# jonathan-innis/karpenter-provider-aws

Hardware: AMD Instinct MI355X
Metric: pods scheduled/sec (Solve, 50k pods × EC2 catalog) (higher is better)
Workload: dtype int64; 1 GPU; config2: 50000 heterogeneous pods (250 classes) x 918 types x 3 AZ x {spot,on-demand}, 2 NodePools; pods=50000, types=918, parallelism=single

## Files before the change

karpenter-provider-aws_amd/csrc/kp_bound.h:

```cpp
#pragma once
#include <stdint.h>

#if defined(__HIPCC__) || defined(__CUDACC__)
#define KP_BOUND_HD __host__ __device__ inline
#else
#define KP_BOUND_HD inline
#endif

#define KP_BOUND_STRIDE 8
#define KP_NO_BOUND INT64_MAX

KP_BOUND_HD int64_t kp_bound_entry(int64_t max_alloc, bool witness) { return witness ? max_alloc : KP_NO_BOUND; }

KP_BOUND_HD bool kp_bound_rejects(int64_t bound, int64_t total, int64_t pod) {
    return pod > 0 && bound != KP_NO_BOUND && total > bound - pod;
}
```

karpenter-provider-aws_amd/csrc/kp_ffd.h:

```cpp
#pragma once
#include <hip/hip_runtime.h>
#include <stdint.h>

#include <type_traits>

#include "kp_bound.h"
#include "kp_device.h"
#include "kp_eval.h"
#include "kp_gosort.h"
#include "kp_layout.h"

namespace KP_WNS {

#ifdef KP_NO_TOPO
#define KP_TOPO_ON 0
#else
#define KP_TOPO_ON 1
#endif

__device__ __forceinline__ bool ports_meet(const KpDev& d, const uint64_t* m, int c) {
    uint64_t x = 0;
    for (int w = 0; w < d.PW; w++)
        x |= __hip_atomic_load(const_cast<uint64_t*>(m) + w, __ATOMIC_RELAXED, __HIP_MEMORY_SCOPE_AGENT) &
             d.cls_ports[(size_t)c * d.PW + w];
// ... 294 lines not shown
}

__device__ inline void topo_record_quick(const KpDev& d, FfdShared& S, int c, int nc, int tmpl, uint64_t born, int lane) {
    const bool hit = S.tr_cls == c;
    const int r0 = hit ? 0 : d.cls_troff[c], nr = hit ? S.tr_n : d.cls_troff[c + 1] - r0;
    const bool keep = !hit && nr <= KP_SNAP_ROWS;
    for (int base = 0; base < nr; base += 64) {
        const int i = base + lane;
        KpTopoRec R{};
        uint32_t fl = 0;
        uint64_t w = 0;
        bool live = false;
        if (i < nr) {
            R = hit ? S.tr_R[i] : d.cls_tre[r0 + i];
            if (keep) S.tr_R[i] = R;
            live = !((R.skip >> tmpl) & 1ull) && (R.late < 0 || ((born >> R.late) & 1ull));
            if (live && !(R.flags & 8)) {
                fl = d.nc_hdr[(size_t)nc * d.K + R.key].flags;
                w = d.nc_words[(size_t)nc * d.DW + d.woff[R.key]];
                const int type = R.flags & TG_TYPE;
                const bool inv = (R.flags >> 2) & 1;
                live = (fl & RF_DEF) && !(!inv && type != 2 && ((fl & RF_CMP) || __popcll(w) != 1));
            }
        }
        for (uint64_t m = ballot(live); m; m &= m - 1) {
            const int j = __ffsll((unsigned long long)m) - 1;
            const int g = rl32(R.g, j), flags = rl32(R.flags, j), key = rl32(R.key, j);
            if (flags & 8) {
                if (lane == 0) {
                    const int old = atomicAdd(&d.tg_hcnt[(size_t)(-1 - key) * d.HN + d.E + nc], 1);
                    if (old == 0) atomicAdd(&d.tg_pos[g], 1);
                }
                continue;
            }
            const uint64_t wv = rl64(w, j);
            if ((wv >> lane) & 1ull) atomicAdd(&d.tg_cnt[(size_t)g * 64 + lane], 1);
            if (lane == 0 && wv) atomicOr((unsigned long long*)&d.tg_known[g], (unsigned long long)wv);
        }
    }
    if (keep && lane == 0) {
        S.tr_n = nr;
        S.tr_cls = c;
    }
    asm volatile("s_waitcnt vmcnt(0)" ::: "memory");
}

#define KP_CAND_VIRT 0x40000000
#ifndef KP_BOUND_SWEEP
#define KP_BOUND_SWEEP 0
#endif
#ifndef KP_BOUND_IDLE_WAVE
#define KP_BOUND_IDLE_WAVE 1
#endif
template <bool PROF>
static __device__ __attribute__((noinline)) int bound_round(const int64_t* __restrict__ nc_bound,
                                                            const int64_t* __restrict__ nc_req,
                                                            int R, int A,
                                                            FfdShared& S, uint32_t* key, const uint16_t* ord, int buf,
                                                            int cnt, int sdone, int r) {
    static_assert(KP_NWAVES <= 8 && KP_LDS_AXES <= KP_BOUND_STRIDE && KP_BOUND_STRIDE == 8, "lane = 8 candidate + axis");
    const int lane = (int)__lane_id(), ci = lane >> 3, ai = lane & 7;
    const bool v = ci < cnt && ai < A;
    const int nc = ord[S.cand_pos[buf][ci < cnt ? ci : 0]];
    const int64_t b = v ? __hip_atomic_load(const_cast<int64_t*>(&nc_bound[(size_t)nc * KP_BOUND_STRIDE + ai]), __ATOMIC_RELAXED,
                                            __HIP_MEMORY_SCOPE_AGENT) : KP_NO_BOUND;
    const int64_t tot = v ? ld_req(&nc_req[(size_t)nc * R + r]) : 0;
    const uint64_t m = ballot(v && kp_bound_rejects(b, tot, S.pod_req[r]));
    if (!m) return 0;
    uint64_t vm = 0;
    for (int i = 0; i < 8; i++)
        if ((m >> (8 * i)) & 0xFFull) vm |= 1ull << i;
    const int nv = __popcll(vm);
    const int p = lane < cnt ? S.cand_pos[buf][lane] : 0;
    const bool rej = (vm >> lane) & 1ull;
    if (nv == cnt && !sdone) {
        if (rej) key[p] |= 0x80000000u;
        if (lane == 0) {
            S.st[ST_NC_EVALS] += cnt;
            S.st[ST_BOUND_SKIPS] += cnt;
            if (PROF) S.st[ST_BOUND_ALLV]++;
            S.fwd = 1;
        }
        return 1;
    }
    if (rej) S.cand_pos[buf][lane] = p | KP_CAND_VIRT;
    if (PROF && lane == 0) S.st[nv == cnt ? ST_BOUND_ALLV : ST_BOUND_MIXED]++;
    return 0;
}
template <bool TOPO, bool PORTS = false, bool BOUND = false, bool PROF = false>
__device__ inline bool collect_candidates(const KpDev& d, FfdShared& S,
                                          std::conditional_t<PORTS || BOUND, uint32_t*, const uint32_t*> key,
                                          const uint16_t* ord, const uint8_t* stmpl, uint64_t tol, int N, int start, int buf,
                                          int lane, int pc = -1, bool bound = false) {
    int pos = start;
    bool marked = false;
    for (;;) {
        int cnt = 0, next = N;
        const int tp_n = TOPO ? S.tp_n : 0;
        const int L = tp_n ? d.topo_cands : KP_NWAVES;
        while (pos < N) {
            const int p = pos + lane;
            bool c = p < N && !(key[p] >> 31);
            if (c) c = (tol >> stmpl[ord[p]]) & 1ull;
            if (PORTS && pc >= 0) {
                const bool meet = c && ports_meet(d, d.nc_ports + (size_t)ord[p] * d.PW, pc);
                if constexpr (PORTS)
                    if (meet) key[p] |= 0x80000000u;
                marked |= ballot(meet) != 0;
                c = c && !meet;
            }
            if (tp_n && c) c = topo_prefilter_pass(d, S, ord[p]);
            const uint64_t m0 = __ballot(c);
            if (tp_n && m0 && cnt + __popcll(m0) < L) {
                const int rank = cnt + __popcll(m0 & ((1ull << lane) - 1ull));
                if (c) S.cand_pos[buf][rank] = p;
                cnt += __popcll(m0);
                pos += 64;
                if (lane == 0) {
                    S.n_cand[buf] = cnt;
                    S.scan_next[buf] = pos < N ? pos : N;
                    S.scan_done[buf] = pos >= N;
                }
                return marked;
            }
            const uint64_t m = __ballot(c);
            const int rank = cnt + __popcll(m & ((1ull << lane) - 1ull));
            if (c && rank < L) S.cand_pos[buf][rank] = p;
            const int tot = cnt + __popcll(m);
            if (tot >= L) {
                const uint64_t last = __ballot(c && rank == L - 1);
                next = pos + __ffsll((unsigned long long)last);
                cnt = L;
                break;
            }
            cnt = tot;
            pos += 64;
        }
        const bool sdone = (cnt < L) || next >= N;
        if constexpr (BOUND) {
            if (bound && cnt > 0 && d.lds_A > 0) {
                __builtin_amdgcn_fence(__ATOMIC_SEQ_CST, "wavefront");
                if (bound_round<PROF>(d.nc_bound, d.nc_req, d.R, d.lds_A, S, key, ord,
                                            buf, cnt, sdone, act_axis(d, lane & 7))) {
                    marked = true;
                    pos = next;
                    continue;
                }
            }
        }
        if (lane == 0) {
            S.n_cand[buf] = cnt;
            S.scan_next[buf] = cnt == L ? next : N;
            S.scan_done[buf] = sdone;
        }
        return marked;
    }
}

static __device__ __attribute__((noinline)) void bound_row_store(const KpDev* __restrict__ dp, const int64_t* alloc,
                                                                 const WaveScratch& ws, int nc, int fresh) {
    static_assert(KP_LDS_AXES < KP_BOUND_STRIDE, "the row's last entry holds the walk's first step");
    const KpDev& d = *dp;
    const int lane = (int)__lane_id();
    const int A = d.lds_A, TP = d.lds_tpad;
    const uint16_t* const rank = d.alloc_rank;
    int64_t* const row = d.nc_bound + (size_t)nc * KP_BOUND_STRIDE;
    int64_t mx[KP_LDS_AXES];
#if KP_BOUND_SWEEP
    const int start = 0, first = 0;
    for (int ai = 0; ai < KP_LDS_AXES; ai++) {
        mx[ai] = KP_NO_BOUND;
        if (ai >= A) continue;
        int64_t m = INT64_MIN;
        for (int w = 0; w < d.TW; w++)
            if ((ws.opts[w] >> lane) & 1ull) {
                const int64_t av = alloc[ai * TP + w * 64 + lane];
                m = av > m ? av : m;
            }
        mx[ai] = wave_max64(m);
    }
#else
    int t[KP_LDS_AXES];
#pragma unroll
    for (int ai = 0; ai < KP_LDS_AXES; ai++) {
        mx[ai] = KP_NO_BOUND;
        t[ai] = ai < A ? (int)rank[ai * TP + lane] : 0xFFFF;
    }
    const int start = fresh ? 0 : (int)__hip_atomic_load(&row[KP_BOUND_STRIDE - 1], __ATOMIC_RELAXED, __HIP_MEMORY_SCOPE_AGENT);
    int base = start * 64;
    if (start > 0) {
#pragma unroll
        for (int ai = 0; ai < KP_LDS_AXES; ai++) t[ai] = ai < A ? (int)rank[ai * TP + base + lane] : 0xFFFF;
    }
    uint32_t pending = (1u << A) - 1u;
    int first = -1;
    while (base < TP) {
#pragma unroll
        for (int ai = 0; ai < KP_LDS_AXES; ai++)
            if ((pending >> ai) & 1u) {
                const uint64_t m = ballot(t[ai] < TP && ((ws.opts[t[ai] < TP ? t[ai] >> 6 : 0] >> (t[ai] & 63)) & 1ull));
                if (m) {
                    mx[ai] = alloc[ai * TP + rl32(t[ai], __ffsll((unsigned long long)m) - 1)];
                    pending &= ~(1u << ai);
                    if (first < 0) first = base >> 6;
                }
            }
        base += 64;
        if (!pending || base >= TP) break;
#pragma unroll
        for (int ai = 0; ai < KP_LDS_AXES; ai++) t[ai] = ((pending >> ai) & 1u) ? (int)rank[ai * TP + base + lane] : 0xFFFF;
    }
#endif
    int64_t mine = KP_NO_BOUND;
#pragma unroll
    for (int ai = 0; ai < KP_LDS_AXES; ai++)
        if (lane == ai) mine = mx[ai];
    if (lane < A)
        __hip_atomic_store(&row[lane], kp_bound_entry(mine, ws.hr[lane] >= 0), __ATOMIC_RELAXED, __HIP_MEMORY_SCOPE_AGENT);
    if (lane == KP_BOUND_STRIDE - 1)
        __hip_atomic_store(&row[lane], (int64_t)(first < 0 ? start : first), __ATOMIC_RELAXED, __HIP_MEMORY_SCOPE_AGENT);
}

__device__ __forceinline__ uint64_t limit_filter(const KpDev& d, int j, uint64_t o, int lane) {
    return lane < d.TW ? o & d.tmpl_lmask[(size_t)j * d.TW + lane] : o;
}

__device__ inline void limit_mask_update(const KpDev& d, int j, int lane) {
    uint32_t lm = 0;
    for (int r = 0; r < d.R; r++)
        if (d.limit_set[(size_t)j * d.R + r]) lm |= 1u << r;
    uint64_t mine = ~0ull;
    for (int w = 0; w < d.TW && lm; w++) {
        const int t = w * 64 + lane;
        bool keep = t < d.T;
        for (uint32_t m = lm; m && keep; m &= m - 1) {
            const int r = __ffs(m) - 1;
            keep = d.cap[(size_t)r * d.T + t] <= ld_req(&d.remaining[(size_t)j * d.R + r]);
        }
        const uint64_t nb = ballot(keep);
        if (lane == w) mine = nb;
    }
    if (lane < d.TW) d.tmpl_lmask[(size_t)j * d.TW + lane] = mine;
}

__device__ __forceinline__ long long prof_clock(bool prof) { return prof ? __builtin_amdgcn_s_memtime() : 0; }


__device__ __forceinline__ void commit_reservations(const KpDev& d, int32_t* rcap, const WaveScratch& ws, int nc,
                                                    bool fresh, int* rel_flag, int lane) {
    const int RW = d.ro_ridw;
    if (lane < RW) {
        uint64_t* hp = d.nc_held + (size_t)nc * RW + lane;
        const uint64_t old = fresh ? 0ull : ld_u64(hp), nh = ws.minbits[lane];
        for (uint64_t x = nh & ~old; x; x &= x - 1) rcap[lane * 64 + __ffsll((unsigned long long)x) - 1]--;
        for (uint64_t x = old & ~nh; x; x &= x - 1)
            if (rcap[lane * 64 + __ffsll((unsigned long long)x) - 1]++ == 0) *rel_flag = 1;
        __hip_atomic_store(hp, nh, __ATOMIC_RELAXED, __HIP_MEMORY_SCOPE_AGENT);
    }
    if (lane == 0) __hip_atomic_store(&d.nc_rlive[nc], ws.rlive, __ATOMIC_RELAXED, __HIP_MEMORY_SCOPE_AGENT);
}
__device__ __forceinline__ uint64_t held_word(const KpDev& d, int nc, int lane) {
    return lane < d.ro_ridw ? ld_u64(&d.nc_held[(size_t)nc * d.ro_ridw + lane]) : 0ull;
}

template <bool VOL = false>
static __device__ __attribute__((noinline)) int existing_topo_scan(const KpDev* __restrict__ dp, FfdShared& S, int pod, int lane) {
    const KpDev& d = *dp;
    const int K = d.K;
    const int c = S.cur_cls;
    int vs = 0;
    if constexpr (VOL)
        if (d.VD > 0) vs = __builtin_amdgcn_readfirstlane(d.shape_vs[d.pod_shape[pod]]);
    const bool cons = (d.cls_flags[c] & CF_TOPO_CONS) != 0;
// ... 1259 lines not shown
                    const int i = atomicAdd(&trace[0], 1);
                    {
                        int* e = trace + 1 + 6 * (i % KP_TRACE_N);
                        e[0] = pod;
                        e[1] = nc;
                        e[2] = ok;
                        e[3] = S.ws[wave].memo_ok | (fast << 1) | ((RESV ? ld_i32(&d.nc_rlive[nc]) : 0) << 2);
                        e[4] = S.cand_pos[b][ci];
                        e[5] = (int)(rl64(a.held, 0) & 0xFFFFFFFFu);
                    }
                }
                if (lane == 0) {
                    S.fastp[b][ci] = fast;
                    S.acc[b][ci] = ok;
                    if (!ok && S.ws[wave].memo_ok) {
                        skey[S.cand_pos[b][ci]] |= 0x80000000u;
                        S.any_rej = 1;
                    }
                    if (!ok && !S.ws[wave].memo_ok) S.rej_volatile = 1;
                    if (fast) atomicAdd((unsigned long long*)&S.st[ST_WITNESS_MISS], 1ull);
                }
            }
            __syncthreads();
            const int nc_ = S.n_cand[b];
            for (int w = f0; w < nc_; w++)
                if (S.acc[b][w]) {
                    win = w;
                    break;
                }
            if (tid == 0) S.st[ST_NC_EVALS] += nc_ > f0 ? nc_ - f0 : 0;
            if (win >= 0 || S.scan_done[b]) break;
            if (wave == 0 &&
                collect_candidates<TOPO_ON, PORTS, BOUND, PROF>(d, S, skey, sord, stmpl, S.topo_pod ? d.tol[S.cur_cls] : ~0ull, S.N,
                                                                      S.scan_next[b], b ^ 1, lane,
                                                                      (PORTS && (S.CC.flags & CF_PORTS)) ? S.cur_cls : -1,
                                                                      BOUND && !(S.CC.flags & CF_TOPO)) && lane == 0)
                S.any_rej = 1;
            __syncthreads();
            round++;
        }
        long long c_ev = 0;
        if (tid == 0 && prof) {
            const long long t1 = __builtin_amdgcn_s_memtime();
            S.st[ST_CYC_SCAN] += t1 - c_slow;
            S.st[ST_SEG + 3] += t1 - c_ev0;
            c_ev = t1;
        }
        if (prof && tid == 0 && !S.topo_pod)
            S.st[ST_SLOW_WHY + (win < 0 ? 7 : (round == 0 && win == 0) ? 5 : 6)]++;
        if (win >= 0) {
            const int cw = (team || team_won) ? 0 : win - (round == 0 ? first : 0);
            if (BOUND && wave == (cw + KP_BOUND_IDLE_WAVE) % KP_NWAVES)
            {
                bound_row_store(d.self, E.alloc, S.ws[(team || team_won) ? wave : cw], sord[S.cand_pos[round & 1][win]], 0);
                asm volatile("s_waitcnt vmcnt(0)" ::: "memory");
            }
            if (wave == cw) {
                const int pos = S.cand_pos[round & 1][win];
                const int nc = sord[pos];
                if (!S.fastp[round & 1][win]) {
                    commit_reqs(d, S.CC, S.ws[cw], nc, lane);
                    if (RESV && d.resv_on) commit_reservations(d, sRcap, S.ws[cw], nc, false, &S.rel_flag, lane);
                }
                if (PREF && d.best_effort) {
                    asm volatile("s_waitcnt vmcnt(0)" ::: "memory");
                    commit_min_relax(d, S.ws[cw], nc, lane);
                }
                if (TOPO_ON && (S.CC.flags & CF_TOPO))
                    topo_record(d, S.CC, S.ws[cw], d.nc_hdr + (size_t)nc * K, d.nc_words + (size_t)nc * d.DW,
                                d.E + nc, d.nc_tmpl[nc], true, lane, -1, nullptr, S.born);
                if (lane < TW) d.nc_opts[(size_t)nc * TW + lane] = S.ws[cw].opts[lane];
                if (PORTS && (S.CC.flags & CF_PORTS)) nodeclaim_ports_commit(d, nc, S.cur_cls, false, 0, lane);
                if (lane < R && S.pod_req[lane])
                    atomicAdd((unsigned long long*)&d.nc_req[(size_t)nc * R + lane], (unsigned long long)S.pod_req[lane]);
                if (lane < A && nc < NQ) shr[lane * NQ + nc] = S.ws[cw].hr[lane];
                if (lane == 0) {
                    slast[nc] = (uint16_t)S.cur_cls;
                    skey[pos]++;
                    S.dirty_kind = 1;
                    S.dirty_pos = pos;
                    S.scan_start = ((S.CC.flags & CF_TOPO) || S.rej_volatile) ? 0 : pos;
                    if (trace && S.cur_cls == -2 - d.trace_pod && pod <= d.trace_max) {
                        const int i = atomicAdd(&trace[0], 1);
                        {
                            int* e = trace + 1 + 6 * (i % KP_TRACE_N);
                            e[0] = pod;
                            e[1] = -1000 - nc;
                            e[2] = S.scan_start;
                            e[3] = S.rej_volatile;
                            e[4] = pos;
                            e[5] = 0;
                        }
                    }
                    d.pod_result[pod] = nc;
                    d.pod_order[pod] = S.seq++;
                }
                asm volatile("s_waitcnt vmcnt(0)" ::: "memory");
            }
        } else {
            const long long c_t = prof_clock(prof);
            auto commit_tmpl = [&](int jj, int cw) {
                const int n = S.N;
                for (int k = lane; k < K; k += 64) d.nc_hdr[(size_t)n * K + k] = d.cls_hdr[(size_t)(d.C + jj) * K + k];
                for (int i = lane; i < d.DW; i += 64)
                    d.nc_words[(size_t)n * d.DW + i] = d.cls_words[(size_t)(d.C + jj) * d.DW + i];
                asm volatile("s_waitcnt vmcnt(0)" ::: "memory");
                commit_reqs(d, S.CC, S.ws[cw], n, lane);
                if (PREF && d.best_effort) {
                    asm volatile("s_waitcnt vmcnt(0)" ::: "memory");
                    commit_min_relax(d, S.ws[cw], n, lane);
                }
                if (RESV && d.resv_on) commit_reservations(d, sRcap, S.ws[cw], n, true, &S.rel_flag, lane);
                if (TOPO_ON && (S.CC.flags & CF_TOPO))
                    topo_record(d, S.CC, S.ws[cw], d.cls_hdr + (size_t)(d.C + jj) * K,
                                d.cls_words + (size_t)(d.C + jj) * d.DW, d.E + n, jj, true, lane, -1, nullptr,
                                S.born);
                if (lane < TW) d.nc_opts[(size_t)n * TW + lane] = S.ws[cw].opts[lane];
                if (PORTS) nodeclaim_ports_commit(d, n, S.cur_cls, true, jj, lane);
                for (int r = lane; r < R; r += 64)
                    __hip_atomic_store(&d.nc_req[(size_t)n * R + r], d.daemon[(size_t)jj * R + r] + S.pod_req[r],
                                       __ATOMIC_RELAXED, __HIP_MEMORY_SCOPE_AGENT);
                if (lane < A && n < NQ) shr[lane * NQ + n] = S.ws[cw].hr[lane];
                if (BOUND) bound_row_store(d.self, E.alloc, S.ws[cw], n, 1);
                for (int r = 0; r < R; r++) {
                    if (!d.limit_set[(size_t)jj * R + r]) continue;
                    int64_t mx = INT64_MIN;
                    for (int w2 = 0; w2 < TW; w2++) {
                        const uint64_t ow = S.ws[cw].opts[w2];
                        if ((ow >> lane) & 1ull) {
                            const int64_t cp = d.cap[(size_t)r * T + w2 * 64 + lane];
                            mx = cp > mx ? cp : mx;
                        }
                    }
                    mx = wave_max64(mx);
                    if (lane == 0) d.remaining[(size_t)jj * R + r] -= mx;
                }
                asm volatile("s_waitcnt vmcnt(0)" ::: "memory");
                limit_mask_update(d, jj, lane);
                if (lane == 0) {
                    slast[n] = (uint16_t)S.cur_cls;
                    stmpl[n] = (uint8_t)jj;
                    d.nc_tmpl[n] = jj;
                    sord[n] = (uint16_t)n;
                    skey[n] = 1;
                    S.N = n + 1;
                    S.dirty_kind = 2;
                    S.dirty_pos = n;
                    d.pod_result[pod] = n;
                    d.pod_order[pod] = S.seq++;
                }
                asm volatile("s_waitcnt vmcnt(0)" ::: "memory");
            };
            int twin = -1;
            if (KP_TEAM_TMPL && (!RESV || KP_TEAM_TMPL_RESV) && !TOPO && d.team_first) {
                for (int j = 0; j < d.NT; j++) {
                    uint64_t o = (lane < TW && d.tmpl_ok[j]) ? d.tmpl_opts[(size_t)j * TW + lane] : 0;
                    o = limit_filter(d, j, o, lane);
                    if (PORTS && (S.CC.flags & CF_PORTS) && ports_meet(d, d.tmpl_ports + (size_t)j * d.PW, S.cur_cls)) o = 0;
                    if (!ballot(o != 0)) continue;
                    EvalIn a;
                    a.Ahdr = d.cls_hdr + (size_t)(d.C + j) * K;
                    a.Aw = d.cls_words + (size_t)(d.C + j) * d.DW;
                    a.opts = o;
                    a.base_req = d.daemon + (size_t)j * R;
                    a.pod_req = S.pod_req;
                    a.tmpl = j;
                    a.compat = true;
                    a.force_off = false;
                    a.prof = nullptr;
                    a.host = d.E + S.N;
                    a.held = 0;
                    TeamBuf* const tbuf = &S.team[tjoins & 1];
                    const bool ok = (TOPO_ON && (S.CC.flags & CF_TOPO_CONS))
                                        ? eval_wave<true, RESV, true, PREF, false, true, PROF>(d, E, S.CC, a, S.ws[wave], lane, tbuf,
                                                                                         wave, KP_NWAVES, &tjoins)
                                        : eval_wave<false, RESV, true, PREF, false, true, PROF>(d, E, S.CC, a, S.ws[wave], lane,
                                                                                          tbuf, wave, KP_NWAVES, &tjoins);
                    if (tid == 0) S.st[ST_TMPL_EVALS]++;
                    if (trace && pod == d.trace_pod && tid == 0) {
                        const int i = atomicAdd(&trace[0], 1);
                        int* e = trace + 1 + 6 * (i % KP_TRACE_N);
                        e[0] = -1;
                        e[1] = -1 - j;
                        e[2] = ok;
                        e[3] = S.ws[0].memo_ok;
                        e[4] = e[5] = 0;
                    }
                    if (ok) {
                        twin = j;
                        break;
                    }
                }
                if (twin >= 0 && (S.N >= NCMAX || S.N >= d.NCcap)) {
                    if (tid == 0) S.err = 1;
                    twin = -1;
                }
                if (twin >= 0 && wave == 0) commit_tmpl(twin, 0);
            } else
            for (int tb = 0; tb < d.NT; tb += KP_NWAVES) {
                const int j = tb + wave;
                if (j < d.NT) {
                    uint64_t o = (lane < TW && d.tmpl_ok[j]) ? d.tmpl_opts[(size_t)j * TW + lane] : 0;
                    o = limit_filter(d, j, o, lane);
                    if (PORTS && (S.CC.flags & CF_PORTS) && ports_meet(d, d.tmpl_ports + (size_t)j * d.PW, S.cur_cls)) o = 0;
                    bool ok = false;
                    if (ballot(o != 0)) {
                        EvalIn a;
                        a.Ahdr = d.cls_hdr + (size_t)(d.C + j) * K;
                        a.Aw = d.cls_words + (size_t)(d.C + j) * d.DW;
                        a.opts = o;
                        a.base_req = d.daemon + (size_t)j * R;
                        a.pod_req = S.pod_req;
                        a.tmpl = j;
                        a.compat = true;
                        a.force_off = false;
                        a.prof = nullptr;
                        a.host = d.E + S.N;
                        a.held = 0;
                        ok = (TOPO_ON && (S.CC.flags & CF_TOPO_CONS)) ? eval_wave<true, RESV, true, PREF, false, false, PROF>(d, E, S.CC, a, S.ws[wave], lane)
                                                         : eval_wave<false, RESV, true, PREF, false, false, PROF>(d, E, S.CC, a, S.ws[wave], lane);
                    }
                    if (trace && pod == d.trace_pod && lane == 0) {
                        const int i = atomicAdd(&trace[0], 1);
                        {
                            int* e = trace + 1 + 6 * (i % KP_TRACE_N);
                            e[0] = -1;
                            e[1] = -1 - j;
                            e[2] = ok;
                            e[3] = S.ws[wave].memo_ok;
                            e[4] = e[5] = 0;
                        }
                    }
                    if (lane == 0) S.tacc[wave] = ok;
                }
                __syncthreads();
                for (int w = 0; w < KP_NWAVES && tb + w < d.NT; w++)
                    if (S.tacc[w]) {
                        twin = w;
                        break;
                    }
                if (tid == 0) S.st[ST_TMPL_EVALS] += (d.NT - tb < KP_NWAVES ? d.NT - tb : KP_NWAVES);
                if (twin >= 0 && (S.N >= NCMAX || S.N >= d.NCcap)) {
                    if (tid == 0) S.err = 1;
                    twin = -1;
                    break;
                }
                if (twin >= 0) {
                    if (wave == twin) {
                        const int jj = tb + wave;
                        const int n = S.N;
                        for (int k = lane; k < K; k += 64) d.nc_hdr[(size_t)n * K + k] = d.cls_hdr[(size_t)(d.C + jj) * K + k];
                        for (int i = lane; i < d.DW; i += 64)
                            d.nc_words[(size_t)n * d.DW + i] = d.cls_words[(size_t)(d.C + jj) * d.DW + i];
                        asm volatile("s_waitcnt vmcnt(0)" ::: "memory");
                        commit_reqs(d, S.CC, S.ws[wave], n, lane);
                        if (PREF && d.best_effort) {
                            asm volatile("s_waitcnt vmcnt(0)" ::: "memory");
                            commit_min_relax(d, S.ws[wave], n, lane);
                        }
                        if (RESV && d.resv_on) commit_reservations(d, sRcap, S.ws[wave], n, true, &S.rel_flag, lane);
                        if (TOPO_ON && (S.CC.flags & CF_TOPO))
                            topo_record(d, S.CC, S.ws[wave], d.cls_hdr + (size_t)(d.C + jj) * K,
                                        d.cls_words + (size_t)(d.C + jj) * d.DW, d.E + n, jj, true, lane, -1, nullptr,
                                        S.born);
                        if (lane < TW) d.nc_opts[(size_t)n * TW + lane] = S.ws[wave].opts[lane];
                        if (PORTS) nodeclaim_ports_commit(d, n, S.cur_cls, true, jj, lane);
                        for (int r = lane; r < R; r += 64)
                            __hip_atomic_store(&d.nc_req[(size_t)n * R + r], d.daemon[(size_t)jj * R + r] + S.pod_req[r],
                                               __ATOMIC_RELAXED, __HIP_MEMORY_SCOPE_AGENT);
                        if (lane < A && n < NQ) shr[lane * NQ + n] = S.ws[wave].hr[lane];
                        if (BOUND) bound_row_store(d.self, E.alloc, S.ws[wave], n, 1);
                        for (int r = 0; r < R; r++) {
                            if (!d.limit_set[(size_t)jj * R + r]) continue;
                            int64_t mx = INT64_MIN;
                            for (int w2 = 0; w2 < TW; w2++) {
                                const uint64_t ow = S.ws[wave].opts[w2];
                                if ((ow >> lane) & 1ull) {
                                    const int64_t cp = d.cap[(size_t)r * T + w2 * 64 + lane];
                                    mx = cp > mx ? cp : mx;
                                }
                            }
                            mx = wave_max64(mx);
                            if (lane == 0) d.remaining[(size_t)jj * R + r] -= mx;
                        }
                        asm volatile("s_waitcnt vmcnt(0)" ::: "memory");
                        limit_mask_update(d, jj, lane);
                        if (lane == 0) {
                            slast[n] = (uint16_t)S.cur_cls;
                            stmpl[n] = (uint8_t)jj;
                            d.nc_tmpl[n] = jj;
                            sord[n] = (uint16_t)n;
                            skey[n] = 1;
                            S.N = n + 1;
                            S.dirty_kind = 2;
                            S.dirty_pos = n;
                            d.pod_result[pod] = n;
                            d.pod_order[pod] = S.seq++;
                        }
                        asm volatile("s_waitcnt vmcnt(0)" ::: "memory");
                    }
                    break;
                }
                __syncthreads();
            }
            if (tid == 0) {
                if (prof) S.st[ST_CYC_TMPL] += __builtin_amdgcn_s_memtime() - c_t;
                if (twin < 0) {
                    const int tail = (S.qhead + S.qcount) % P;
                    d.qbuf[tail] = pod;
                    S.qcount++;
                    const int nx = (PREF && d.relax_next) ? d.relax_next[S.cur_cls] : -1;
                    if (nx >= 0) {
                        d.pod_cls[pod] = nx;
                        d.pod_shape[pod] = d.shape_next[S.prev_shape];
                        S.epoch++;
                        S.relaxed = 1;
                        if (d.tg_late) S.born = topo_birth(d, S.born, d.cls_birth[nx]);
                    } else {
                        d.last_len[pod] = S.qcount;
                        if (PREF && d.last_ep) d.last_ep[pod] = S.epoch;
                    }
                }
            }
        }
// ... 68 lines not shown
```

karpenter-provider-aws_amd/csrc/kp_host.cpp:

```cpp
#include <hip/hip_runtime.h>

#include <arpa/inet.h>

#include <algorithm>
#include <array>
#include <atomic>
#include <cfloat>
#include <chrono>
#include <cstdint>
#include <cstdio>
#include <cstring>
#include <map>
#include <set>
#include <memory>
#include <string>
#include <condition_variable>
#include <functional>
#include <mutex>
#include <thread>
#include <unordered_map>
#include <vector>

#include "../../include/kpsim.h"
#include "kp_gosort_host.h"
// ... 394 lines not shown
    DBuf<kp_probe_result> d_probe_out;
    DBuf<int32_t> d_rec_i;
    DBuf<int64_t> d_prof_probe;
    DBuf<ReqHdr> d_rec_hdr;
    DBuf<uint64_t> d_rec_words;
    DBuf<int32_t> d_mut_s, d_mut_m, d_ov_slot, d_pov_node, d_vov_node, d_vov_cnt;
    DBuf<uint64_t> d_vov_mask;
    std::vector<int32_t> h_pod_vs;
    std::vector<int64_t> h_vol_enc;
    DBuf<uint64_t> d_pov_mask;
    DBuf<ReqHdr> d_ov_hdr;
    DBuf<uint64_t> d_ov_words;
    int cons_n_mut = 0;
    uint64_t cons_gen = 0;
    uint64_t pass_gen = ~0ull;
    int pass_mode = -1;
    std::vector<kp_probe_result> pass_rows;
    uint64_t rec_gen = ~0ull;
    int rec_mode = -1, rec_probe = -1;
    kp_probe_result rec_row{};
    int32_t rec_ri[4 + 64 + 1] = {};
    std::vector<ReqHdr> rec_h;
    std::vector<uint64_t> rec_w;
    int64_t n_pass_launches = 0, n_readbacks = 0;
    KpCons cons{};
    bool cons_prepared = false;
    bool cons_prep_valid = false;
    int32_t* cons_q0 = nullptr;
    int cons_max_candidates = 100, cons_n_pending = 0;
    std::vector<int32_t> cons_off;
    double cons_ms[3] = {};
    int64_t cons_stats[CS_COUNT] = {};
    bool has_reserved = false, launch_ok = true;
    std::string solve_unsupported;
    bool ro_ok = true;
    std::string ro_why;
    bool wide_resvid = false;
    bool resvid_rows = false;
    std::vector<int32_t> ro_type, ro_zone, ro_zid, ro_rid, ro_ridv, ro_rtype;
    std::vector<int32_t> ro_rid_vid;
    std::vector<uint64_t> ro_avail;
    std::vector<int32_t> ro_off;
    std::vector<uint32_t> type_ro;
    std::vector<int32_t> rcap0;
    std::vector<double> ro_price;
    ResvTab h_ro{};
    std::vector<ResvTab> h_ro_up;
    DBuf<ResvTab> d_ro;
    DBuf<int32_t> d_ro_type, d_ro_zone, d_ro_zid, d_ro_rid, d_ro_ridv, d_ro_rtype, d_ro_rid_vid;
    DBuf<uint64_t> d_ro_avail;
    DBuf<uint32_t> d_type_ro;
    DBuf<uint64_t> d_nc_held;
    DBuf<int32_t> d_rcap0, d_nc_rlive;
    DBuf<uint16_t> d_alloc_rank;
    DBuf<int64_t> d_nc_bound;
    DBuf<double> d_ro_price;
    DBuf<int32_t> d_trace;
    std::string launch_err;
    std::vector<std::vector<std::pair<int, int>>> type_single;
    int ct_vid[3] = {-1, -1, -1};
    std::vector<int32_t> l_off_begin, l_off_val, l_ct, l_rt, l_rcap;
    std::vector<double> l_price;
    std::vector<uint8_t> l_avail, l_exotic;
    DBuf<int32_t> d_l_off_begin, d_l_off_val, d_l_ct, d_l_rt, d_l_rcap, d_l_hdr, d_l_types;
    DBuf<uint64_t> d_l_over;
    DBuf<double> d_l_price;
    DBuf<uint8_t> d_l_avail, d_l_exotic;
    DBuf<KlReq> d_l_req;
    DBuf<KlKey> d_l_keys[2];
    DBuf<KlMinKey> d_l_mins[2];
    DBuf<uint64_t> d_l_words[2];
    DBuf<int64_t> d_l_rq;
    PinBuf<KlReq> p_l_req;
    PinBuf<int64_t> p_l_rq;
    PinBuf<KlKey> p_l_keys[2];
    PinBuf<KlMinKey> p_l_mins[2];
    PinBuf<uint64_t> p_l_words[2], p_l_over;
    PinBuf<int32_t> p_l_hdr, p_l_types;
    PinBuf<int32_t> p_pcls, p_pshape;
    PinBuf<int64_t> p_preq, p_fields;
    WorkerPool pool;
    double launch_ms[6] = {};
    int launch_nsub = 0;
    double launch_busy_ms = 0;
    hipEvent_t lev[3 * KL_MAX_SUB] = {};
    int tg_G = 0, tg_HG = 0;
    DBuf<int4> d_tg_info;
    DBuf<int32_t> d_tg_hrow, d_tg_owner, d_tg_pol, d_tg_cnt0, d_tg_cnt, d_tg_hcnt0, d_tg_hcnt, d_tg_pos0, d_tg_pos,
        d_cls_tcoff, d_cls_tc, d_cls_troff, d_cls_tr;
    DBuf<KpTopoCons> d_cls_tce;
    DBuf<int2> d_tce_hosts;
    DBuf<int2> d_tg_frow;
    DBuf<int32_t> d_tg_late;
    DBuf<uint64_t> d_cls_birth, d_born_s, d_born_m, d_late_sib;
    DBuf<int32_t> d_late_grp;
    int tg_nlate = 0;
    bool tg_var = false;
    std::vector<uint64_t> h_late_sib;
    std::vector<uint64_t> h_cls_birth;
    DBuf<KpTopoRec> d_cls_tre;
    DBuf<uint64_t> d_tg_known0, d_tg_known;
    DBuf<uint8_t> d_cls_kneutral, d_vrank;
    std::vector<std::array<int, 3>> cons_extra;
    int cons_extra_ncand = 0;
    std::vector<int> cons_pend;
    bool cons_topo = false;
// ... 2657 lines not shown
    d.E = E;
    d.EW = EW;
    DEV(ex_hdr0); DEV(ex_words0); DEV(ex_hdr); DEV(ex_words); DEV(ex_avail); DEV(ex_req); DEV(ex_head); DEV(ex_static);
    DEV(XT); DEV(ex_tol); DEV(cls_xkoff); DEV(cls_xkeys);
    d.ex_mayfix = se.mayfix ? 1 : 0;
    d.P = P;
    DEV(pod_cls); DEV(pod_shape);
    const bool relax = !c->pref.relax_next.empty();
    d.relax_next = relax ? c->d_relax_next.p : nullptr;
    d.shape_next = relax ? c->d_shape_next.p : nullptr;
    d.pod_cls0 = relax ? c->d_pod_cls0.p : nullptr;
    d.pod_shape0 = relax ? c->d_pod_shape0.p : nullptr;
    d.last_ep = relax ? c->d_last_ep.p : nullptr;
    d.best_effort = c->best_effort ? 1 : 0;
    DEV(pod_req);
    d.queue0 = nullptr;
    d.NCcap = NCcap;
    DEV(nc_hdr); DEV(nc_words); DEV(nc_opts); DEV(nc_req); DEV(nc_tmpl); DEV(empty_hdr); DEV(empty_words); DEV(qbuf);
    DEV(last_len); DEV(pod_result); DEV(pod_order); DEV(nc_count); DEV(nc_npods); DEV(nc_slice_pos); DEV(nc_nopts);
    DEV(nc_valid);
    d.M = M;
    DEV(nc_types); DEV(nc_ntypes); DEV(stats); DEV(err);
    d.G = G;
    d.key_host = se.th.key_host;
    DEV(tg_info); DEV(tg_hrow); DEV(tg_owner); DEV(tg_pol); DEV(tg_frow);
    d.tg_late = c->tg_nlate > 0 ? c->d_tg_late.p : nullptr;
    d.cls_birth = c->tg_nlate > 0 ? c->d_cls_birth.p : nullptr;
    d.late_sib = c->tg_var ? c->d_late_sib.p : nullptr;
    d.late_grp = c->tg_var ? c->d_late_grp.p : nullptr;
    DEV(tg_cnt); DEV(tg_known); DEV(tg_hcnt); DEV(tg_pos); DEV(cls_tcoff); DEV(cls_tc); DEV(cls_troff); DEV(cls_tr);
    DEV(cls_tce); DEV(tce_hosts); DEV(cls_tre); DEV(cls_kneutral); DEV(vrank);
    for (int ai = 0; ai < KP_LDS_AXES; ai++) {
        int sh = 0;
        if (ai < d.n_active) {
            int64_t mx = 0;
            for (int t = 0; t < T; t++) mx = std::max(mx, c->alloc_rt[(size_t)d.active_axes[ai] * T + t]);
            while ((mx >> sh) > 0x3FFFFFFF) sh++;
        }
        d.qshift[ai] = sh;
    }
    {
        const int TP = (T + 63) / 64 * 64, ns = std::min(d.n_active, KP_LDS_AXES);
        static_assert(KP_MAX_TYPES < 0xFFFF, "alloc_rank holds type ids as u16, 0xFFFF is its padding");
        std::vector<uint16_t> rank((size_t)std::max(ns, 1) * TP, 0xFFFF);
        std::vector<int> ord(T);
        for (int ai = 0; ai < ns; ai++) {
            const int64_t* al = &c->alloc_rt[(size_t)d.active_axes[ai] * T];
            for (int t = 0; t < T; t++) ord[t] = t;
            std::stable_sort(ord.begin(), ord.end(), [&](int x, int y) { return al[x] > al[y]; });
            for (int t = 0; t < T; t++) rank[(size_t)ai * TP + t] = (uint16_t)ord[t];
        }
        HIPCHK(c->d_alloc_rank.upload(rank, s));
        d.alloc_rank = c->d_alloc_rank.p;
    }
    d.ro = c->h_ro.n > 0 ? c->d_ro.p : nullptr;
    DEV(type_ro); DEV(ro_price);
    d.ro_n = c->h_ro.n;
    d.ro_w = c->h_ro.w;
    d.ro_nrid = c->h_ro.nrid;
    d.ro_ridw = c->h_ro.ridw;
    d.resv_on = (c->reserved_capacity && c->h_ro.n > 0) ? 1 : 0;
    DEV(rcap0); DEV(nc_held); DEV(nc_rlive); DEV(nc_bound);
    d.alloc_act = nullptr;
    if (NCcap > KP_NC_FIRST || T > 1024) {
        const int TP = (T + 63) / 64 * 64, ns = std::min(d.n_active, KP_LDS_AXES);
        std::vector<int64_t> act((size_t)std::max(ns, 1) * TP, 0);
        for (int ai = 0; ai < ns; ai++)
            for (int t = 0; t < T; t++) act[(size_t)ai * TP + t] = c->alloc_rt[(size_t)d.active_axes[ai] * T + t];
        HIPCHK(c->d_alloc_stage.upload(act, s));
        d.alloc_act = c->d_alloc_stage.p;
        HIPCHK(c->d_g_key.ensure(NCcap));
        HIPCHK(c->d_g_ord.ensure(NCcap));
        HIPCHK(c->d_g_last.ensure(NCcap));
        HIPCHK(c->d_g_tmpl.ensure(NCcap));
        DEV(g_key); DEV(g_ord); DEV(g_last); DEV(g_tmpl);
    }
    return KP_OK;
}
#undef DEV

static kp_status solve_diag_switches(kp_ctx* ctx, const kp_solve_input* in, SolveEnc& se) {
    KpDev& d = ctx->dev;
    d.profile = getenv("KPSIM_PROFILE") ? 1 : 0;
    {
        const int nw = ctx->tg_G > 0 ? KP_NWAVES_TOPO : KP_NWAVES;
        d.topo_cands = getenv("KPSIM_TOPO_CANDS") ? std::max(1, std::min(nw, atoi(getenv("KPSIM_TOPO_CANDS")))) : nw;
    }
    d.team_eval = getenv("KPSIM_NO_TEAM") ? 0 : 1;
    d.noop_quick = getenv("KPSIM_NO_NOOP") ? 0 : 1;
    d.team_first = getenv("KPSIM_NO_TEAM_FIRST") ? 0 : 1;
    d.block_sort = getenv("KPSIM_NO_BLOCK_SORT") ? 0 : 1;
    d.trace_pod = getenv("KPSIM_TRACE_POD") ? atoi(getenv("KPSIM_TRACE_POD"))
                  : getenv("KPSIM_TRACE_CLASS") ? -2 - atoi(getenv("KPSIM_TRACE_CLASS")) : -1;
    d.trace_max = getenv("KPSIM_TRACE_MAXPOD") ? atoi(getenv("KPSIM_TRACE_MAXPOD")) : INT32_MAX;
    d.trace = nullptr;
    if (d.trace_pod != -1) {
        HIPCHK(ctx->d_trace.ensure(1 + 6 * KP_TRACE_N + 3 + 2 * 4096));
        d.trace = ctx->d_trace.p;
    }
    return KP_OK;
}


static kp_status solve_plan_lds(kp_ctx* ctx, const kp_solve_input* in, SolveEnc& se) {
    KpDev& d = ctx->dev;
    if (!kp_ffd_plan_lds(d, KP_LDS_BYTES)) return fail(ctx, KP_E_UNSUPPORTED, "FFD kernel LDS plan exceeds 160 KB");
// ... 2037 lines not shown
```

karpenter-provider-aws_amd/csrc/kp_layout.h:

```cpp
#pragma once
#include <stdint.h>

#ifndef KP_MAX_TYPES
#define KP_MAX_TYPES 2048
#endif
#define KP_TW_MAX (KP_MAX_TYPES / 64)
#define KP_DNE_TW 16
#define KP_MAX_NC 65535
#define KP_NC_FIRST 4096
#define KP_MAX_KEYS 96
#define KP_MAX_CLASS_KEYS 32
#define KP_MAX_SLOTS 64
#define KP_MAX_NP 63
#define KP_MAX_R 16
#ifndef KP_NWAVES
#define KP_NWAVES 8
#endif
#ifndef KP_NWAVES_TOPO
#define KP_NWAVES_TOPO 4
#endif
#define KP_WNS_CAT2(n) kp_w##n
#define KP_WNS_CAT(n) KP_WNS_CAT2(n)
#define KP_WNS KP_WNS_CAT(KP_NWAVES)
#define KP_LDS_AXES 6
// ... 189 lines not shown
    int32_t HN;
    int32_t key_host;
    const int4* tg_info;
    const int32_t* tg_hrow;
    const int32_t* tg_owner;
    const int32_t* tg_pol;
    const int2* tg_frow;
    int32_t snap_rows;
    const int32_t* tg_late;
    const uint64_t* cls_birth;
    uint64_t born0;
    const uint64_t* late_sib;
    const int32_t* late_grp;
    int32_t* tg_cnt;
    uint64_t* tg_known;
    int32_t* tg_hcnt;
    int32_t* tg_pos;
    const int32_t* cls_tcoff;
    const int32_t* cls_tc;
    const int32_t* cls_troff;
    const int32_t* cls_tr;
    const uint8_t* cls_kneutral;
    const uint8_t* vrank;
    const struct KpTopoCons* cls_tce;
    const int2* tce_hosts;
    const struct KpTopoRec* cls_tre;

    int32_t lds_ncmax;
    int32_t slice_hbm;
    uint32_t* g_key;
    uint16_t* g_ord;
    uint16_t* g_last;
    uint8_t* g_tmpl;
    int32_t lds_tpad;
    int32_t lds_nstage;
    int32_t lds_A;
    int32_t lds_nq;
    int32_t alloc_global;
    const int64_t* alloc_act;
    int32_t off_key, off_ord, off_last, off_tmpl, off_alloc, off_avail, off_multi, off_ro, off_tsnap, off_hr, off_qw;
    int32_t lds_bytes;
    int32_t qshift[KP_LDS_AXES];

    const ResvTab* ro;
    const uint32_t* type_ro;
    const double* ro_price;
    int32_t ro_n, ro_w, ro_nrid, ro_ridw;
    int32_t ro_stage;
    int32_t resv_on;
    const int32_t* rcap0;
    uint64_t* nc_held;
    int32_t* nc_rlive;
    const uint16_t* alloc_rank;
    int64_t* nc_bound;

    const KpDev* self;

    int32_t PW;
    const uint64_t* cls_ports;
    const uint64_t* tmpl_ports;
    const uint64_t* ex_ports0;
    uint64_t* ex_ports;
    uint64_t* nc_ports;

    int32_t VD, VW;
    const int32_t* shape_vs;
    const int32_t* vs_cnt;
    const uint64_t* vs_mask;
    const uint64_t* drv_mask;
    const int32_t* ex_vlim;
    const int32_t* ex_vcnt0;
    int32_t* ex_vcnt;
    const uint64_t* ex_vmask0;
    uint64_t* ex_vmask;
    const uint8_t* ex_vover;
};

enum {
    ST_POPPED = 0, ST_NC_EVALS, ST_NC_SCANNED, ST_TMPL_EVALS, ST_EXIST_EVALS, ST_SORT_FAST, ST_SORT_FULL,
    ST_BOUND_MIXED, ST_CYC_POP, ST_CYC_SORT, ST_CYC_SCAN, ST_CYC_TMPL, ST_CYC_COMMIT, ST_CYC_SORT_FULL,
    ST_N_INNER = 14, ST_CYC_QINNER, ST_N_MULTI = 22,
    ST_BOUND_SKIPS = 23, ST_BOUND_ALLV = 31,
    ST_EV_REQ = 16, ST_EV_MASK, ST_EV_OFF, ST_EV_TYPES, ST_EV_MIN, ST_EV_CALLS,
    ST_QUICK = 24, ST_SLOW, ST_WITNESS_MISS, ST_CYC_QPOP, ST_CYC_QSCAN, ST_CYC_QCHECK, ST_CYC_QCOMMIT,
    ST_N_NOINV = 32, ST_N_WINMOVE, ST_N_LDSSORT, ST_N_PIVOT, ST_N_WINLOAD, ST_N_FLUSH, ST_N_SHAPE, ST_EXIST_PLACED = 44,
    ST_TOPO_QUICK = 45, ST_CYC_TSETUP, ST_CYC_TSCAN,
    ST_REJ_REQ = 48, ST_REJ_TOPO, ST_REJ_TYPES, ST_REJ_MIN,
    ST_TQ_WHY = 52, ST_SLOW_WHY = 59,
    ST_SEG = 70, ST_TQ_ITERS = 75, ST_TQ_CYC = 76,
    ST_HANDOFF = 77, ST_HANDOFF_WB = 43, ST_COUNT = 80
};
```

Measured before the change: 673,300 pods/s.

## Cache per-axis witness types in bound rows and skip unchanged row recomputation

Each nodeclaim bound row now stores a packed tail recording which type was the max-alloc witness on each axis, plus the walk's starting step. On update, the row is skipped when every axis's witness is still among the options and its witness status is unchanged. Template commits on the team path move the bound-row computation onto an idle wave and start the walk at a host-precomputed first step per template. This adds a host-side precompute and a tighter row-layout constraint, and it risks stale bounds if the skip test misses a case.

```diff
diff --git a/karpenter-provider-aws_amd/csrc/kp_bound.h b/karpenter-provider-aws_amd/csrc/kp_bound.h
--- a/karpenter-provider-aws_amd/csrc/kp_bound.h
+++ b/karpenter-provider-aws_amd/csrc/kp_bound.h
@@ -10,6 +10,34 @@
 #define KP_BOUND_STRIDE 8
 #define KP_NO_BOUND INT64_MAX
 
+#define KP_BOUND_TAIL_AXES 6
+#define KP_BOUND_NO_TYPE 0xFFFFu
+struct KpBoundTail {
+    uint64_t lo, hi;
+};
+KP_BOUND_HD KpBoundTail kp_bound_tail_empty(unsigned step) {
+    return KpBoundTail{~0ull, 0x0000FFFFFFFFFFFFull | ((uint64_t)(step & 0xFFFFu) << 48)};
+}
+KP_BOUND_HD void kp_bound_tail_set(KpBoundTail& t, int axis, unsigned type) {
+    uint64_t& w = axis < 4 ? t.lo : t.hi;
+    const int sh = 16 * (axis & 3);
+    w = (w & ~(0xFFFFull << sh)) | ((uint64_t)(type & 0xFFFFu) << sh);
+}
+KP_BOUND_HD unsigned kp_bound_tail_type(uint64_t lo, uint64_t hi, int axis) {
+    return (unsigned)(((axis < 4 ? lo : hi) >> (16 * (axis & 3))) & 0xFFFFu);
+}
+KP_BOUND_HD unsigned kp_bound_tail_step(uint64_t hi) { return (unsigned)(hi >> 48); }
+KP_BOUND_HD int kp_bound_first_step(const uint16_t* rank, int TP, const uint64_t* set) {
+    for (int k = 0; k < TP; k++) {
+        const unsigned t = rank[k];
+        if (t != KP_BOUND_NO_TYPE && ((set[t >> 6] >> (t & 63)) & 1ull)) return k >> 6;
+    }
+    return TP >> 6;
+}
+KP_BOUND_HD bool kp_bound_axis_kept(unsigned type, const uint64_t* opts, int nw, int64_t entry, bool witness) {
+    return type < (unsigned)(64 * nw) && ((opts[type >> 6] >> (type & 63)) & 1ull) && ((entry != KP_NO_BOUND) == witness);
+}
+
 KP_BOUND_HD int64_t kp_bound_entry(int64_t max_alloc, bool witness) { return witness ? max_alloc : KP_NO_BOUND; }
 
 KP_BOUND_HD bool kp_bound_rejects(int64_t bound, int64_t total, int64_t pod) {
diff --git a/karpenter-provider-aws_amd/csrc/kp_ffd.h b/karpenter-provider-aws_amd/csrc/kp_ffd.h
--- a/karpenter-provider-aws_amd/csrc/kp_ffd.h
+++ b/karpenter-provider-aws_amd/csrc/kp_ffd.h
@@ -370,6 +370,12 @@
 #ifndef KP_BOUND_IDLE_WAVE
 #define KP_BOUND_IDLE_WAVE 1
 #endif
+#ifndef KP_BOUND_ROW_SKIP
+#define KP_BOUND_ROW_SKIP 1
+#endif
+#ifndef KP_BOUND_TMPL_IDLE
+#define KP_BOUND_TMPL_IDLE 1
+#endif
 template <bool PROF>
 static __device__ __attribute__((noinline)) int bound_round(const int64_t* __restrict__ nc_bound,
                                                             const int64_t* __restrict__ nc_req,
@@ -475,17 +481,31 @@
     }
 }
 
+template <bool PROF>
 static __device__ __attribute__((noinline)) void bound_row_store(const KpDev* __restrict__ dp, const int64_t* alloc,
-                                                                 const WaveScratch& ws, int nc, int fresh) {
-    static_assert(KP_LDS_AXES < KP_BOUND_STRIDE, "the row's last entry holds the walk's first step");
+                                                                 const WaveScratch& ws, int nc, int fresh_step, long long* st) {
+    static_assert(KP_LDS_AXES <= KP_BOUND_STRIDE - 2 && KP_LDS_AXES <= KP_BOUND_TAIL_AXES, "the row's last two entries hold its tail");
     const KpDev& d = *dp;
     const int lane = (int)__lane_id();
     const int A = d.lds_A, TP = d.lds_tpad;
     const uint16_t* const rank = d.alloc_rank;
     int64_t* const row = d.nc_bound + (size_t)nc * KP_BOUND_STRIDE;
     int64_t mx[KP_LDS_AXES];
+    int start = fresh_step < 0 ? 0 : fresh_step;
+    if (fresh_step < 0) {
+        const int64_t e = lane < KP_BOUND_STRIDE ? __hip_atomic_load(&row[lane], __ATOMIC_RELAXED, __HIP_MEMORY_SCOPE_AGENT) : 0;
+        const uint64_t lo = rl64((uint64_t)e, KP_BOUND_STRIDE - 2), hi = rl64((uint64_t)e, KP_BOUND_STRIDE - 1);
+#if KP_BOUND_ROW_SKIP
+        const bool kept = lane >= A || kp_bound_axis_kept(kp_bound_tail_type(lo, hi, lane), ws.opts, TP >> 6, e, ws.hr[lane] >= 0);
+        if (!ballot(!kept)) return;
+        if (PROF && lane == 0) atomicAdd((unsigned long long*)&st[ST_BOUND_ROWS], 1ull);
+#endif
+        start = (int)kp_bound_tail_step(hi);
+    }
+    KpBoundTail tail = kp_bound_tail_empty(0);
 #if KP_BOUND_SWEEP
-    const int start = 0, first = 0;
+    const int first = 0;
+    start = 0;
     for (int ai = 0; ai < KP_LDS_AXES; ai++) {
         mx[ai] = KP_NO_BOUND;
         if (ai >= A) continue;
@@ -499,16 +519,11 @@
     }
 #else
     int t[KP_LDS_AXES];
+    int base = start * 64;
 #pragma unroll
     for (int ai = 0; ai < KP_LDS_AXES; ai++) {
         mx[ai] = KP_NO_BOUND;
-        t[ai] = ai < A ? (int)rank[ai * TP + lane] : 0xFFFF;
-    }
-    const int start = fresh ? 0 : (int)__hip_atomic_load(&row[KP_BOUND_STRIDE - 1], __ATOMIC_RELAXED, __HIP_MEMORY_SCOPE_AGENT);
-    int base = start * 64;
-    if (start > 0) {
-#pragma unroll
-        for (int ai = 0; ai < KP_LDS_AXES; ai++) t[ai] = ai < A ? (int)rank[ai * TP + base + lane] : 0xFFFF;
+        t[ai] = (ai < A && base < TP) ? (int)rank[ai * TP + base + lane] : 0xFFFF;
     }
     uint32_t pending = (1u << A) - 1u;
     int first = -1;
@@ -518,7 +533,9 @@
             if ((pending >> ai) & 1u) {
                 const uint64_t m = ballot(t[ai] < TP && ((ws.opts[t[ai] < TP ? t[ai] >> 6 : 0] >> (t[ai] & 63)) & 1ull));
                 if (m) {
-                    mx[ai] = alloc[ai * TP + rl32(t[ai], __ffsll((unsigned long long)m) - 1)];
+                    const int ty = rl32(t[ai], __ffsll((unsigned long long)m) - 1);
+                    mx[ai] = alloc[ai * TP + ty];
+                    kp_bound_tail_set(tail, ai, (unsigned)ty);
                     pending &= ~(1u << ai);
                     if (first < 0) first = base >> 6;
                 }
@@ -529,14 +546,16 @@
         for (int ai = 0; ai < KP_LDS_AXES; ai++) t[ai] = ((pending >> ai) & 1u) ? (int)rank[ai * TP + base + lane] : 0xFFFF;
     }
 #endif
+    tail.hi = (tail.hi & 0x0000FFFFFFFFFFFFull) | ((uint64_t)(unsigned)(first < 0 ? start : first) << 48);
     int64_t mine = KP_NO_BOUND;
 #pragma unroll
     for (int ai = 0; ai < KP_LDS_AXES; ai++)
         if (lane == ai) mine = mx[ai];
     if (lane < A)
         __hip_atomic_store(&row[lane], kp_bound_entry(mine, ws.hr[lane] >= 0), __ATOMIC_RELAXED, __HIP_MEMORY_SCOPE_AGENT);
-    if (lane == KP_BOUND_STRIDE - 1)
-        __hip_atomic_store(&row[lane], (int64_t)(first < 0 ? start : first), __ATOMIC_RELAXED, __HIP_MEMORY_SCOPE_AGENT);
+    if (lane == KP_BOUND_STRIDE - 2 || lane == KP_BOUND_STRIDE - 1)
+        __hip_atomic_store(&row[lane], (int64_t)(lane == KP_BOUND_STRIDE - 2 ? tail.lo : tail.hi), __ATOMIC_RELAXED,
+                           __HIP_MEMORY_SCOPE_AGENT);
 }
 
 __device__ __forceinline__ uint64_t limit_filter(const KpDev& d, int j, uint64_t o, int lane) {
@@ -1902,7 +1921,8 @@
             const int cw = (team || team_won) ? 0 : win - (round == 0 ? first : 0);
             if (BOUND && wave == (cw + KP_BOUND_IDLE_WAVE) % KP_NWAVES)
             {
-                bound_row_store(d.self, E.alloc, S.ws[(team || team_won) ? wave : cw], sord[S.cand_pos[round & 1][win]], 0);
+                bound_row_store<PROF>(d.self, E.alloc, S.ws[(team || team_won) ? wave : cw], sord[S.cand_pos[round & 1][win]], -1,
+                                      S.st);
                 asm volatile("s_waitcnt vmcnt(0)" ::: "memory");
             }
             if (wave == cw) {
@@ -1971,7 +1991,7 @@
                     __hip_atomic_store(&d.nc_req[(size_t)n * R + r], d.daemon[(size_t)jj * R + r] + S.pod_req[r],
                                        __ATOMIC_RELAXED, __HIP_MEMORY_SCOPE_AGENT);
                 if (lane < A && n < NQ) shr[lane * NQ + n] = S.ws[cw].hr[lane];
-                if (BOUND) bound_row_store(d.self, E.alloc, S.ws[cw], n, 1);
+                if (BOUND && !KP_BOUND_TMPL_IDLE) bound_row_store<PROF>(d.self, E.alloc, S.ws[cw], n, 0, S.st);
                 for (int r = 0; r < R; r++) {
                     if (!d.limit_set[(size_t)jj * R + r]) continue;
                     int64_t mx = INT64_MIN;
@@ -2003,6 +2023,7 @@
             };
             int twin = -1;
             if (KP_TEAM_TMPL && (!RESV || KP_TEAM_TMPL_RESV) && !TOPO && d.team_first) {
+                const int n_new = BOUND ? S.N : 0;
                 for (int j = 0; j < d.NT; j++) {
                     uint64_t o = (lane < TW && d.tmpl_ok[j]) ? d.tmpl_opts[(size_t)j * TW + lane] : 0;
                     o = limit_filter(d, j, o, lane);
@@ -2041,9 +2062,13 @@
                         break;
                     }
                 }
-                if (twin >= 0 && (S.N >= NCMAX || S.N >= d.NCcap)) {
+                if (twin >= 0 && ((BOUND ? n_new : S.N) >= NCMAX || (BOUND ? n_new : S.N) >= d.NCcap)) {
                     if (tid == 0) S.err = 1;
                     twin = -1;
+                }
+                if (BOUND && KP_BOUND_TMPL_IDLE && twin >= 0 && wave == KP_BOUND_IDLE_WAVE % KP_NWAVES) {
+                    bound_row_store<PROF>(d.self, E.alloc, S.ws[wave], n_new, d.tmpl_bstep[twin], S.st);
+                    asm volatile("s_waitcnt vmcnt(0)" ::: "memory");
                 }
                 if (twin >= 0 && wave == 0) commit_tmpl(twin, 0);
             } else
@@ -2119,7 +2144,8 @@
                             __hip_atomic_store(&d.nc_req[(size_t)n * R + r], d.daemon[(size_t)jj * R + r] + S.pod_req[r],
                                                __ATOMIC_RELAXED, __HIP_MEMORY_SCOPE_AGENT);
                         if (lane < A && n < NQ) shr[lane * NQ + n] = S.ws[wave].hr[lane];
-                        if (BOUND) bound_row_store(d.self, E.alloc, S.ws[wave], n, 1);
+                        if (BOUND)
+                            bound_row_store<PROF>(d.self, E.alloc, S.ws[wave], n, KP_BOUND_TMPL_IDLE ? d.tmpl_bstep[jj] : 0, S.st);
                         for (int r = 0; r < R; r++) {
                             if (!d.limit_set[(size_t)jj * R + r]) continue;
                             int64_t mx = INT64_MIN;
diff --git a/karpenter-provider-aws_amd/csrc/kp_host.cpp b/karpenter-provider-aws_amd/csrc/kp_host.cpp
--- a/karpenter-provider-aws_amd/csrc/kp_host.cpp
+++ b/karpenter-provider-aws_amd/csrc/kp_host.cpp
@@ -470,6 +470,7 @@
     DBuf<uint32_t> d_type_ro;
     DBuf<uint64_t> d_nc_held;
     DBuf<int32_t> d_rcap0, d_nc_rlive;
+    DBuf<int32_t> d_tmpl_bstep;
     DBuf<uint16_t> d_alloc_rank;
     DBuf<int64_t> d_nc_bound;
     DBuf<double> d_ro_price;
@@ -3233,6 +3234,15 @@
         }
         HIPCHK(c->d_alloc_rank.upload(rank, s));
         d.alloc_rank = c->d_alloc_rank.p;
+        std::vector<int32_t> bstep(std::max(se.NT, 1), 0);
+        for (int j = 0; j < se.NT && ns > 0; j++) {
+            int st = TP / 64;
+            for (int ai = 0; ai < ns; ai++)
+                st = std::min(st, kp_bound_first_step(&rank[(size_t)ai * TP], TP, &se.rows[(size_t)j * ctx->TW]));
+            bstep[j] = st < TP / 64 ? st : 0;
+        }
+        HIPCHK(c->d_tmpl_bstep.upload(bstep, s));
+        d.tmpl_bstep = c->d_tmpl_bstep.p;
     }
     d.ro = c->h_ro.n > 0 ? c->d_ro.p : nullptr;
     DEV(type_ro); DEV(ro_price);
diff --git a/karpenter-provider-aws_amd/csrc/kp_layout.h b/karpenter-provider-aws_amd/csrc/kp_layout.h
--- a/karpenter-provider-aws_amd/csrc/kp_layout.h
+++ b/karpenter-provider-aws_amd/csrc/kp_layout.h
@@ -265,6 +265,7 @@
     uint64_t* nc_held;
     int32_t* nc_rlive;
     const uint16_t* alloc_rank;
+    const int32_t* tmpl_bstep;
     int64_t* nc_bound;
 
     const KpDev* self;
@@ -294,6 +295,7 @@
     ST_BOUND_MIXED, ST_CYC_POP, ST_CYC_SORT, ST_CYC_SCAN, ST_CYC_TMPL, ST_CYC_COMMIT, ST_CYC_SORT_FULL,
     ST_N_INNER = 14, ST_CYC_QINNER, ST_N_MULTI = 22,
     ST_BOUND_SKIPS = 23, ST_BOUND_ALLV = 31,
+    ST_BOUND_ROWS = 46,
     ST_EV_REQ = 16, ST_EV_MASK, ST_EV_OFF, ST_EV_TYPES, ST_EV_MIN, ST_EV_CALLS,
     ST_QUICK = 24, ST_SLOW, ST_WITNESS_MISS, ST_CYC_QPOP, ST_CYC_QSCAN, ST_CYC_QCHECK, ST_CYC_QCOMMIT,
     ST_N_NOINV = 32, ST_N_WINMOVE, ST_N_LDSSORT, ST_N_PIVOT, ST_N_WINLOAD, ST_N_FLUSH, ST_N_SHAPE, ST_EXIST_PLACED = 44,
@@ -303,3 +305,4 @@
     ST_SEG = 70, ST_TQ_ITERS = 75, ST_TQ_CYC = 76,
     ST_HANDOFF = 77, ST_HANDOFF_WB = 43, ST_COUNT = 80
 };
+static_assert(ST_BOUND_ROWS == ST_CYC_TSETUP, "ST_BOUND_ROWS shares the topology setup slot");
```

Result: faster. 713,800 pods/s (median of 6 runs) (+6.0%).
